# microsoft/SEAL

Measured on AMD Instinct MI355X. Metric: CKKS multiply+relinearize+rescale ciphertexts/sec @ N=2^16, L=16, higher is better.
Workload: dtype u64

## Files before the change

### seal_amd/csrc/ntt2_kernels.hip

```cpp
#include "ntt2_device.h"
#include <algorithm>
#include <atomic>
#include <mutex>
#include <cstdlib>
#include <type_traits>
#include <vector>



namespace sealhip
{
    namespace
    {

        template <bool FP, int D1, int ICLS = 0, bool PACK = false>
        __device__ __forceinline__ void fwd_p1_body(const FwdArgs &a, unsigned prime, unsigned comp, unsigned outer, uint64_t *lds, unsigned tile)
        {
            typedef Field<FP> F;
            typedef Geo<D1> G;
            const unsigned tid = threadIdx.x, cg = tile;
            const typename F::Mod m = F::make_mod(ld_uniform_mod(&a.t.mods[prime]), ld_uniform_fpd(&a.t.fpd[prime]));
            const typename F::tw_t *tab = tw_table<FP>(a.t, false, prime);
            SrcMap sm{ 0, 0, 0, 0 };
            const uint64_t *in0;
            size_t in_stride;
            if (a.src)
            {
                in0 = a.src + ((size_t)(comp % a.src_ncomp) << G::n);
                in_stride = a.src_outer_stride;
                sm.mode = a.src_mode;
                sm.half = a.src_half;
                sm.src_q = a.src_q;
                sm.fix = a.src_mode >= 2 ? a.src_fix[comp] : 0;
            }
            else
            {
                in0 = a.data + ((size_t)comp << G::n);
                in_stride = a.outer_stride;
            }
            const unsigned c = tid & (G::C - 1), rbl = tid >> G::LC;
            in0 += cg * G::C + c;
            TwRegs<FP> tw;
            p1_load_tw<FP, D1>(tw, tab, tid);
            uint64_t nxt[16];
            auto fetch = [&](unsigned z) {
                const uint64_t *in = in0 + (size_t)z * in_stride;
#pragma unroll
                for (int e = 0; e < 16; e++)
                {
                    const unsigned ra = e >> (4 - G::rA), rbh = e & ((1 << (4 - G::rA)) - 1);
                    const unsigned R = ra * 16 + (rbh << G::rA) + rbl;
#ifdef SEALHIP_P1_NOLOAD
                    nxt[e] = (uint64_t)(tid * 16 + e + z * 4099u + R) & 0xFFFFFFFFFFFFull;
#else
                    nxt[e] = a.src ? in[(size_t)R * 256] : mid_ld<16>(in + (size_t)R * 256);
#endif
                }
            };
            const unsigned ostride = gridDim.z;
            fetch(outer);
            for (; outer < a.nouter; outer += ostride)
            {
                typename F::elem x[16];
#pragma unroll
                for (int e = 0; e < 16; e++)
                    x[e] = map_src<FP>(nxt[e], sm, m);
                prio_phase<2>();
                if (outer + ostride < a.nouter)
                    fetch(outer + ostride);
                prio_phase<1>();
                uint64_t *mid_tr = a.mid + (((size_t)outer * a.ncomp + comp) << G::n);
#ifndef SEALHIP_P1_PLAIN_LEAN
#define SEALHIP_P1_PLAIN_LEAN 0
#endif
                p1_tile<FP, D1, 256, SEALHIP_P1_PLAIN_LEAN && FP && G::rA == 4, ICLS, PACK>(x, m, tab, tw, lds, mid_tr, cg, tid);
            }
        }

        template <int D1, int CLS>
#ifndef SEALHIP_PACK_WAVES_P1
#define SEALHIP_PACK_WAVES_P1 3
#endif
        __global__ void __launch_bounds__(kThreads, CLS == 5 ? SEALHIP_PACK_WAVES_P1 : CLS == 1 ? SEALHIP_FP_WAVES_P1 : 2) ntt2_fwd_p1(FwdArgs a)
        {
            HIP_DYNAMIC_SHARED(uint64_t, lds)
            const Blk blk = spread_blocks();
            const unsigned comp = blk.y + a.comp0, outer = blk.z;
            const unsigned prime = SHL_UNIFORM(a.comp_prime ? a.comp_prime[comp] : a.prime_first + comp);
            if constexpr (CLS == 5)
                fwd_p1_body<true, D1, 0, D1 == 8>(a, prime, comp, outer, lds, blk.tile);
            else if constexpr (CLS == 1)
                fwd_p1_body<true, D1>(a, prime, comp, outer, lds, blk.tile);
            else if constexpr (CLS == 0)
                with_int_class(a.t, prime, [&](auto ic) { fwd_p1_body<false, D1, decltype(ic)::value>(a, prime, comp, outer, lds, blk.tile); });
            else if (a.t.fpd[prime].qi)
                fwd_p1_body<true, D1>(a, prime, comp, outer, lds, blk.tile);
            else
                fwd_p1_body<false, D1, 2>(a, prime, comp, outer, lds, blk.tile);
        }

        template <bool FP, int D1, bool HOIST = false, bool HOIST_LDS = false, int ICLS = 0, bool PACK = false>
        __device__ __forceinline__ void fwd_p2_body(const FwdArgs &a, unsigned prime, unsigned comp, unsigned outer, uint64_t *lds, unsigned tile)
        {
            typedef Field<FP> F;
            typedef Geo<D1> G;
            const unsigned tid = threadIdx.x, hg = tile;
            const typename F::Mod m = F::make_mod(ld_uniform_mod(&a.t.mods[prime]), ld_uniform_fpd(&a.t.fpd[prime]));
            const typename F::tw_t *tab = tw_table<FP>(a.t, false, prime);
            const uint64_t *mid0 = a.mid + ((size_t)comp << G::n) + ((size_t)hg << 12) + mid_lane(tid);
            uint64_t *lds_wave = lds + (tid >> 6) * (4 * kRowWords);
            uint64_t nxt[16];
            auto fetch = [&](unsigned z) {
                const uint64_t *mp = mid0 + (((size_t)z * a.ncomp) << G::n);
#pragma unroll
                for (int e = 0; e < 16; e++)
                    nxt[e] = mid_ld<4>(mp + e * kMidRow);
            };
            constexpr bool packed = PACK;
            static_assert(!PACK || (FP && D1 == 8), "the packed intermediate is defined for the double-precision pass at N = 2^16");
            [[maybe_unused]] const uint64_t *pk0 = a.mid + ((size_t)comp << G::n) + (size_t)(hg * 16 + (tid >> 4)) * kPackBlock + (tid & 15);
            [[maybe_unused]] auto fetch_packed = [&](unsigned z) {
                const uint64_t *mp = pk0 + (((size_t)z * a.ncomp) << G::n);
#if SEALHIP_PACK_VEC16
                const uint64_t *m2 = mp + (tid & 15);
#pragma unroll
                for (int j = 0; j < 6; j++)
                    mid_ld2<4>(m2 + j * 32, nxt[2 * j], nxt[2 * j + 1]);
                nxt[12] = mid_ld<4>(mp + 192);
#else
#pragma unroll
                for (int k = 0; k < 13; k++)
                    nxt[k] = mid_ld<4>(mp + k * 16);
#endif
            };
            const unsigned ostride = gridDim.z;
            TwRegs<FP> pre_a, pre_b;
            const typename F::tw_t *twa = nullptr;
            if constexpr (HOIST_LDS)
            {
                static_assert(FP, "double-precision back end only");
                double *la = reinterpret_cast<double *>(lds + kLds2Words);
                stage_twa<D1>(la, tab, hg, tid);
                twa = la;
                const unsigned h = hg * 16 + (tid >> 4), v = tid & 15;
                load_tw<FP, 4>(pre_b, tab, [&](int t) { return (1u << (D1 + 4 + t)) + ((h * 16 + v) << t); });
                __syncthreads();
            }
            else if constexpr (HOIST)
                p2_load_tw<FP, D1>(pre_a, pre_b, tab, hg, tid);
            if constexpr (packed)
                fetch_packed(outer);
            else
                fetch(outer);
            for (; outer < a.nouter; outer += ostride)
            {
// ... 116 lines not shown
            const int mode = t2.x.halves_added ? 3 : 2;
            const SrcMap s1{ mode, a.src_half, a.src_q, a.src_fix[comp] }, s2{ mode, t2.x.src2_half, t2.x.src2_q, t2.x.src2_fix[comp] };
            const ShoupOp pm = t2.x.pmul[comp];
            const uint64_t q = a.t.mods[prime].q;
            const unsigned c = tid & (G::C - 1), rbl = tid >> G::LC;
            const size_t col = (size_t)cg * G::C + c;
            TwRegs<FP> tw;
            p1_load_tw<FP, D1>(tw, tab, tid);
            const unsigned ostride = gridDim.z;
            for (; outer < a.nouter; outer += ostride)
            {
                const uint64_t *in1 = a.src + (size_t)outer * a.src_outer_stride + col;
                const uint64_t *in2 = ((outer & 1) ? t2.x.src2_1 : t2.x.src2_0) + (size_t)(outer >> 1) * t2.x.src2_stride + col;
                uint64_t n1[16], n2[16];
#pragma unroll
                for (int e = 0; e < 16; e++)
                {
                    const unsigned ra = e >> (4 - G::rA), rbh = e & ((1 << (4 - G::rA)) - 1);
                    const unsigned R = ra * 16 + (rbh << G::rA) + rbl;
                    n1[e] = in1[(size_t)R * 256];
                    n2[e] = in2[(size_t)R * 256];
                }
                typename F::elem x[16];
                if constexpr (FP)
                {
                    const double pinv = pm.w > q / 2 ? -(double)(q - pm.w) : (double)pm.w;
                    const double f1 = fp_from_u52(s1.fix), f2 = fp_from_u52(s2.fix);
                    const bool u_small = !(s2.src_q >> 52);
#pragma unroll
                    for (int e = 0; e < 16; e++)
                    {
                        const uint64_t r1 = mode == 3 ? n1[e] : csub(n1[e] + s1.half, s1.src_q), r2 = mode == 3 ? n2[e] : csub(n2[e] + s2.half, s2.src_q);
                        const double v = F::from_any(r1, m) + f1, u = (u_small ? fp_from_u52(r2) : F::from_any(r2, m)) + f2;
                        x[e] = fp_mulmod(v, pinv, m.q, m.qinv) + u;
                        F::fix(x[e], m);
                    }
                }
                else
                {
#pragma unroll
                    for (int e = 0; e < 16; e++)
                    {
                        const typename F::elem v = map_src<FP>(n1[e], s1, m), u = map_src<FP>(n2[e], s2, m);
                        x[e] = mul_shoup(v, pm.w, pm.wq, q) + u;
                    }
                }
                uint64_t *mid_tr = a.mid + (((size_t)outer * a.ncomp + comp) << G::n);
                p1_tile<FP, D1, 256, FP && G::rA == 4, ICLS>(x, m, tab, tw, lds, mid_tr, cg, tid);
            }
        }

        template <bool FP, int D1, int ICLS>
        __device__ __forceinline__ void tail2_p2_body(const Tail2Args &t2, unsigned prime, unsigned comp, unsigned outer, uint64_t *lds, unsigned tile)
        {
            typedef Field<FP> F;
            typedef Geo<D1> G;
            const FwdArgs &a = t2.f;
            const unsigned tid = threadIdx.x, hg = tile;
            const typename F::Mod m = F::make_mod(ld_uniform_mod(&a.t.mods[prime]), ld_uniform_fpd(&a.t.fpd[prime]));
            const typename F::tw_t *tab = tw_table<FP>(a.t, false, prime);
            const uint64_t *mid0 = a.mid + ((size_t)comp << G::n) + ((size_t)hg << 12) + mid_lane(tid);
            uint64_t *lds_wave = lds + (tid >> 6) * (4 * kRowWords);
            const uint64_t q = a.t.mods[prime].q;
            const ShoupOp mul = a.epi_mul[comp], pm = t2.x.pmul[comp];
            [[maybe_unused]] const double pm_fp = pm.w > q / 2 ? -(double)(q - pm.w) : (double)pm.w;
            [[maybe_unused]] const double mul_fp = mul.w > q / 2 ? -(double)(q - mul.w) : (double)mul.w;
            const size_t row0 = ((size_t)comp << G::n) + ((size_t)(hg * 16 + (tid >> 6) * 4) << 8);
            uint64_t nxt[16];
            auto fetch = [&](unsigned z) {
                const uint64_t *mp = mid0 + (((size_t)z * a.ncomp) << G::n);
#pragma unroll
                for (int e = 0; e < 16; e++)
                    nxt[e] = mid_ld<4>(mp + e * kMidRow);
            };
            const unsigned ostride = gridDim.z;
            fetch(outer);
            for (; outer < a.nouter; outer += ostride)
            {
                typename F::elem x[16];
#pragma unroll
                for (int e = 0; e < 16; e++)
                    x[e] = F::unraw(nxt[e]);
                if (outer + ostride < a.nouter)
                    fetch(outer + ostride);
                const uint64_t *A = a.epi_a + (size_t)outer * a.epi_a_stride + row0;
                const uint64_t *C = ((outer & 1) ? t2.x.c1 : t2.x.c0) + (size_t)(outer >> 1) * t2.x.c_stride + row0;
                const bool folded = t2.x.a_has_c;
                uint64_t av[16], cv[16];
#pragma unroll
                for (int k = 0; k < 16; k++)
                {
                    const unsigned off = (k >> 2) * 256 + (k & 3) * 64 + (tid & 63);
                    av[k] = mid_ld<16>(A + off);
                    cv[k] = folded ? 0 : mid_ld<16>(C + off);
                }
                p2_tile<FP, D1, false, false, false, false, false, ICLS, kP1Out<ICLS, D1>>(x, m, tab, nullptr, nullptr, lds_wave, hg, tid);
                uint64_t val[16];
                uint64_t *O = ((outer & 1) ? a.epi_out1 : a.epi_out0) + (size_t)(outer >> 1) * a.epi_out_stride + row0;
                if constexpr (FP)
                {
#pragma unroll
                    for (int e = 0; e < 16; e++)
                        val[e] = F::raw(x[e]);
                    emit_rows_k(val, lds_wave, tid, [&](int k, unsigned off, uint64_t tv) {
                        const double s = folded ? fp_from_u52(av[k]) : fp_mulmod(fp_from_u52(av[k]), pm_fp, m.q, m.qinv) + fp_from_u52(cv[k]);
                        const double r = fp_mulmod(s - fp_from_bits(tv), mul_fp, m.q, m.qinv);
                        O[off] = fp_to_canon(fp_fix(r, m.q, m.qinv), m);
                    });
                }
                else
                {
#pragma unroll
                    for (int e = 0; e < 16; e++)
                        val[e] = fwd_out_lazy<FP, ICLS, kP2Out<ICLS, D1>>(x[e], m);
                    emit_rows_k(val, lds_wave, tid, [&](int k, unsigned off, uint64_t tv) {
                        const uint64_t s = folded ? av[k] : add_mod(mul_shoup(av[k], pm.w, pm.wq, q), cv[k], q);
                        O[off] = mul_shoup(s + 4 * q - tv, mul.w, mul.wq, q);
                    });
                }
            }
        }

        template <int D1, int CLS>
        __global__ void __launch_bounds__(kThreads, 2) ntt2_tail2_p1(Tail2Args a)
        {
            HIP_DYNAMIC_SHARED(uint64_t, lds)
            const Blk blk = spread_blocks();
            const unsigned comp = blk.y + a.f.comp0, outer = blk.z;
            const unsigned prime = SHL_UNIFORM(a.f.prime_first + comp);
            if constexpr (CLS == 1)
                tail2_p1_body<true, D1, 0>(a, prime, comp, outer, lds, blk.tile);
            else if constexpr (CLS == 0)
                with_int_class(a.f.t, prime, [&](auto ic) { tail2_p1_body<false, D1, decltype(ic)::value>(a, prime, comp, outer, lds, blk.tile); });
            else if (a.f.t.fpd[prime].qi)
                tail2_p1_body<true, D1, 0>(a, prime, comp, outer, lds, blk.tile);
            else
                tail2_p1_body<false, D1, 2>(a, prime, comp, outer, lds, blk.tile);
        }
        template <int D1, int CLS>
        __global__ void __launch_bounds__(kThreads, 2) ntt2_tail2_p2(Tail2Args a)
        {
            HIP_DYNAMIC_SHARED(uint64_t, lds)
            const Blk blk = spread_blocks();
            const unsigned comp = blk.y + a.f.comp0, outer = blk.z;
            const unsigned prime = SHL_UNIFORM(a.f.prime_first + comp);
            if constexpr (CLS == 1)
                tail2_p2_body<true, D1, 0>(a, prime, comp, outer, lds, blk.tile);
            else if constexpr (CLS == 0)
                with_int_class(a.f.t, prime, [&](auto ic) { tail2_p2_body<false, D1, decltype(ic)::value>(a, prime, comp, outer, lds, blk.tile); });
            else if (a.f.t.fpd[prime].qi)
                tail2_p2_body<true, D1, 0>(a, prime, comp, outer, lds, blk.tile);
            else
                tail2_p2_body<false, D1, 2>(a, prime, comp, outer, lds, blk.tile);
        }

        struct InvArgs
        {
            uint64_t *data;
            size_t outer_stride;
            const uint64_t *src;
            size_t src_outer_stride;
            uint64_t *mid;
            const uint32_t *comp_prime;
            int cls_hint;
            unsigned prime_first;
            unsigned ncomp;
            unsigned comp0;
            unsigned nouter;
            int lazy;
            uint64_t out_add;
            const uint64_t *prod_x, *prod_y;
            unsigned prod_batch, prod_outer0;
            uint64_t *prod_out;
            size_t prod_out_stride;
            uint32_t src_gal;
            NttTables t;
        };

        template <int ICLS>
        constexpr int kInvE1 = inv_phase_exp<ICLS>(0, 4, 0);
        template <int ICLS>
        constexpr int kInvE2 = inv_phase_exp<ICLS>(kInvE1<ICLS>, 4, 0);
        template <int ICLS>
        constexpr int kInvE3 = inv_phase_exp<ICLS>(kInvE2<ICLS>, 4, 0);

        template <bool FP, int D1, int ICLS = 2>
        __device__ __forceinline__ void inv_pa_body(const InvArgs &a, unsigned prime, unsigned comp, unsigned outer, uint64_t *lds, unsigned tile)
        {
            typedef Field<FP> F;
            typedef Geo<D1> G;
            const unsigned tid = threadIdx.x, hg = tile;
            const unsigned v = tid & 15, u = tid >> 4, ul = u & 3;
            const unsigned h = hg * 16 + u;
            const typename F::Mod m = F::make_mod(ld_uniform_mod(&a.t.mods[prime]), ld_uniform_fpd(&a.t.fpd[prime]));
            const typename F::tw_t *tab = tw_table<FP>(a.t, true, prime);
            uint64_t *lds_wave = lds + (tid >> 6) * (4 * kRowWords);
            uint64_t raw[16];
            typename F::elem x[16];
            bool have_x = false;
            const size_t rows = ((size_t)comp << G::n) + ((size_t)(hg * 16 + (tid >> 6) * 4) << 8);
            if (a.prod_x)
            {
                const unsigned go = outer + a.prod_outer0, pp = go / a.prod_batch, b = go - pp * a.prod_batch;
                const size_t plane = (size_t)a.prod_batch * a.src_outer_stride, off = (size_t)b * a.src_outer_stride + rows;
                [[maybe_unused]] const ModDesc md = ld_uniform_mod(&a.t.mods[prime]);
                uint64_t rb[16];
                load_rows(raw, lds_wave, a.prod_x + (pp == 2 ? plane : 0) + off, tid);
                load_rows(rb, lds_wave, a.prod_y + (pp == 0 ? 0 : plane) + off, tid);
                if constexpr (FP)
                {
#pragma unroll
                    for (int e = 0; e < 16; e++)
                        x[e] = fp_mulmod(fp_from_u52(raw[e]), fp_from_u52(rb[e]), m.q, m.qinv);
                    if (pp == 1)
                    {
                        uint64_t rc[16];
                        load_rows(rc, lds_wave, a.prod_x + plane + off, tid);
                        load_rows(rb, lds_wave, a.prod_y + off, tid);
#pragma unroll
                        for (int e = 0; e < 16; e++)
                            x[e] += fp_mulmod(fp_from_u52(rc[e]), fp_from_u52(rb[e]), m.q, m.qinv);
                    }
#pragma unroll
                    for (int e = 0; e < 16; e++)
                        F::fix(x[e], m);
                    if (a.prod_out)
                    {
#pragma unroll
                        for (int e = 0; e < 16; e++)
                            raw[e] = fp_to_canon(x[e], m);
                        store_rows(raw, lds_wave, a.prod_out + (size_t)outer * a.prod_out_stride + rows, tid);
                    }
                    have_x = true;
                }
                else
                {
#pragma unroll
                    for (int e = 0; e < 16; e++)
                        raw[e] = mul_mod(raw[e], rb[e], md);
                    if (pp == 1)
                    {
                        uint64_t rc[16];
                        load_rows(rc, lds_wave, a.prod_x + plane + off, tid);
                        load_rows(rb, lds_wave, a.prod_y + off, tid);
#pragma unroll
                        for (int e = 0; e < 16; e++)
                            raw[e] = add_mod(raw[e], mul_mod(rc[e], rb[e], md), md.q);
                    }
                    if (a.prod_out)
                        store_rows(raw, lds_wave, a.prod_out + (size_t)outer * a.prod_out_stride + rows, tid);
                }
            }
            else if (a.src_gal)
                load_rows_galois(raw, lds_wave, a.src + (size_t)outer * a.src_outer_stride + ((size_t)comp << G::n), (hg * 16 + (tid >> 6) * 4) << 8, a.src_gal, G::n, tid);
            else
                load_rows(raw, lds_wave, a.src + (size_t)outer * a.src_outer_stride + rows, tid);
            if (!have_x)
            {
#pragma unroll
                for (int e = 0; e < 16; e++)
                {
                    x[e] = F::from_canon(raw[e], m);
                    F::fix(x[e], m);
                }
            }
            {
                TwRegs<FP> tw;
                load_tw<FP, 4>(tw, tab, [&](int t) { return (1u << (D1 + 4 + t)) + ((h * 16 + v) << t); });
                phase_inv<FP, 4, 0, ICLS, 0>(x, m, [&](int t, int g) { return tw.get((1 << t) + g); });
            }
#pragma unroll
            for (int e = 0; e < 16; e++)
                F::fix(x[e], m);
#pragma unroll
            for (int e = 0; e < 16; e++)
                lds_wave[ul * kRowWords + v * 18 + e] = F::raw(x[e]);
            __builtin_amdgcn_wave_barrier();
#pragma unroll
            for (int e = 0; e < 16; e++)
                x[e] = F::unraw(lds_wave[ul * kRowWords + e * 18 + v]);
            {
                TwRegs<FP> tw;
                load_tw<FP, 4>(tw, tab, [&](int t) { return (1u << (D1 + t)) + (h << t); });
                phase_inv<FP, 4, 0, ICLS, kInvE1<ICLS>>(x, m, [&](int t, int g) { return tw.get((1 << t) + g); });
            }
#pragma unroll
            for (int e = 0; e < 16; e++)
                F::fix(x[e], m);
            uint64_t *mid_tr = a.mid + (((size_t)outer * a.ncomp + comp) << G::n) + ((size_t)hg << 12);
#pragma unroll
            for (int e = 0; e < 16; e++)
                mid_st<8>(mid_tr + e * 256 + tid, F::raw(x[e]));
        }

        template <int D1, int CLS>
        __global__ void __launch_bounds__(kThreads) ntt2_inv_pa(InvArgs a)
        {
            HIP_DYNAMIC_SHARED(uint64_t, lds)
            const Blk blk = spread_blocks();
            const unsigned comp = blk.y + a.comp0, outer = blk.z;
            const unsigned prime = SHL_UNIFORM(a.comp_prime ? a.comp_prime[comp] : a.prime_first + comp);
            if constexpr (CLS == 1)
                inv_pa_body<true, D1>(a, prime, comp, outer, lds, blk.tile);
            else if constexpr (CLS == 0)
                with_int_class(a.t, prime, [&](auto ic) { inv_pa_body<false, D1, decltype(ic)::value>(a, prime, comp, outer, lds, blk.tile); });
            else if (a.t.fpd[prime].qi)
// ... 1087 lines not shown
            {
                const size_t p = i & (N - 1), slab = i >> n_log;
                const unsigned comp = (unsigned)(slab % L);
                const size_t poly = slab / L, digit = poly >> 1;
                const unsigned k = (unsigned)(poly & 1);
                const size_t hg = p >> 12;
                const unsigned e = (unsigned)(p >> 8) & 15, tid = (unsigned)p & 255;
                size_t nat = (hg << 12) + ((size_t)(tid >> 4) << 8) + ((tid & 15) << 4) + e;
                const uint64_t v = in[(slab << n_log) + nat];
                uint64_t *o = out + ((digit * off[L] + off[comp]) << n_log);
                if (fpd[comp].qi)
                {
                    double d = fp_from_u52(v);
                    if (v > fpd[comp].qi / 2)
                        d -= fpd[comp].q;
                    o[2 * p + k] = fp_to_bits(d);
                }
                else
                {
                    typedef unsigned __int128 u128;
                    const ModDesc md = mods[comp];
                    const u128 vr = (u128)v * md.ratio_hi + (((u128)v * md.ratio_lo) >> 64);
                    uint64_t est = vr > (u128)~(uint64_t)0 ? ~(uint64_t)0 : (uint64_t)vr;
                    u128 rem = ((u128)v << 64) - (u128)est * md.q;
                    while (rem >= md.q)
                    {
                        rem -= md.q;
                        est++;
                    }
                    o += (size_t)k << (n_log + 1);
                    o[2 * p] = v;
                    o[2 * p + 1] = est;
                }
            }
        }

        __global__ void __launch_bounds__(kThreads) key_unlayout_kernel(
            const uint64_t *in, uint64_t *out, const FpDesc *fpd, unsigned L, unsigned n_log, size_t polys)
        {
            __shared__ unsigned off[kMaxKeyComps + 1];
            key_offsets(off, fpd, L);
            const size_t N = (size_t)1 << n_log;
            const size_t total = polys * L * N;
            for (size_t i = blockIdx.x * (size_t)kThreads + threadIdx.x; i < total; i += (size_t)gridDim.x * kThreads)
            {
                const size_t p = i & (N - 1), slab = i >> n_log;
                const unsigned comp = (unsigned)(slab % L);
                const size_t poly = slab / L, digit = poly >> 1;
                const unsigned k = (unsigned)(poly & 1);
                const size_t hg = p >> 12;
                const unsigned e = (unsigned)(p >> 8) & 15, tid = (unsigned)p & 255;
                const size_t nat = (hg << 12) + ((size_t)(tid >> 4) << 8) + ((tid & 15) << 4) + e;
                const uint64_t *o = in + ((digit * off[L] + off[comp]) << n_log);
                uint64_t v;
                if (fpd[comp].qi)
                {
                    double d = fp_from_bits(o[2 * p + k]);
                    if (d < 0)
                        d += fpd[comp].q;
                    v = (uint64_t)d;
                }
                else
                    v = o[((size_t)k << (n_log + 1)) + 2 * p];
                out[(slab << n_log) + nat] = v;
            }
        }

        struct CompRun
        {
            unsigned c0, nc;
            int cls;
        };
        std::vector<CompRun> comp_runs(const NttTables &t, const uint32_t *comp_prime, unsigned prime_first, unsigned ncomp, int cls_hint = -1)
        {
            std::vector<CompRun> runs;
            if (comp_prime && (cls_hint == 0 || cls_hint == 1))
            {
                runs.push_back(CompRun{ 0, ncomp, cls_hint });
                return runs;
            }
            static const bool split = !shl_ab_getenv("SEALHIP_NTT_NOSPLIT");
            unsigned c = 0;
            while (c < ncomp)
            {
                int cls = 2;
                unsigned e = ncomp;
                if (split && !comp_prime && t.fp_host)
                {
                    cls = t.fp_host[prime_first + c] ? 1 : 0;
                    e = c + 1;
                    while (e < ncomp && (t.fp_host[prime_first + e] ? 1 : 0) == cls)
                        e++;
                }
                runs.push_back(CompRun{ c, e - c, cls });
                c = e;
            }
            return runs;
        }

        struct SideStream
        {
            hipStream_t stream = nullptr;
            hipEvent_t fork = nullptr, join = nullptr;
            bool ok = false;
            SideStream()
            {
                ok = !shl_ab_getenv("SEALHIP_NTT_NOFORK") && hipStreamCreateWithFlags(&stream, hipStreamNonBlocking) == hipSuccess &&
                     hipEventCreateWithFlags(&fork, hipEventDisableTiming) == hipSuccess &&
                     hipEventCreateWithFlags(&join, hipEventDisableTiming) == hipSuccess;
            }
        };
        SideStream &side_stream()
        {
            static thread_local SideStream s;
            return s;
        }
        template <class RunFn>
        hipError_t launch_runs(const std::vector<CompRun> &runs, hipStream_t s, RunFn run, bool may_fork = true)
        {
            size_t longest = 0;
            for (size_t i = 1; i < runs.size(); i++)
                if (runs[i].nc > runs[longest].nc)
                    longest = i;
            SideStream &ss = side_stream();
            const bool fork = may_fork && runs.size() > 1 && ss.ok;
            hipError_t e;
            if (fork)
            {
                if ((e = hipEventRecord(ss.fork, s)) != hipSuccess || (e = hipStreamWaitEvent(ss.stream, ss.fork, 0)) != hipSuccess)
                    return e;
                for (size_t i = 0; i < runs.size(); i++)
                    if (i != longest && (e = run(runs[i], ss.stream)) != hipSuccess)
                        return e;
                if ((e = hipEventRecord(ss.join, ss.stream)) != hipSuccess)
                    return e;
            }
            for (size_t i = 0; i < runs.size(); i++)
                if ((!fork || i == longest) && (e = run(runs[i], s)) != hipSuccess)
                    return e;
            if (fork && (e = hipStreamWaitEvent(s, ss.join, 0)) != hipSuccess)
                return e;
            return hipSuccess;
        }

#ifndef SEALHIP_FUSED_FORK14
#define SEALHIP_FUSED_FORK14 1
#endif
        inline bool fused_int()
        {
            static const bool on = !shl_ab_getenv("SEALHIP_NTT_NOFUSED_INT");
            return on;
        }

        template <int D1>
        hipError_t launch_fwd(const FwdArgs &a, unsigned nouter, hipStream_t s)
        {
            typedef Geo<D1> G;
            unsigned per = G::TILES * a.ncomp;
#ifndef SEALHIP_NTT_WG_TARGET
#define SEALHIP_NTT_WG_TARGET 8192
#endif
            unsigned chunks = (SEALHIP_NTT_WG_TARGET + per - 1) / per;
            if (const char *f = shl_ab_getenv("SEALHIP_NTT_CHUNKS"))
                chunks = (unsigned)std::atoi(f) ? (unsigned)std::atoi(f) : 1;
            if (chunks > nouter)
                chunks = nouter;
            if (chunks > 65535)
                chunks = 65535;
            size_t l1 = G::rA > 0 ? G::lds1_words * 8 : 8;
            bool fused = false;
            unsigned fchunks = 1;
            if constexpr (D1 == 5 || D1 == 6)
            {
                static const bool fused_ok = !shl_ab_getenv("SEALHIP_NTT_NOFUSED");
                if (fused_ok && (!a.src || a.src_mode == 0) && a.epi == 0)
                {
                    static bool raised = false;
                    if (!raised)
                    {
                        if (hipFuncSetAttribute(reinterpret_cast<const void *>(&ntt2_fwd_fused2<D1, 1>), hipFuncAttributeMaxDynamicSharedMemorySize, (int)FusedGeo<D1>::lds_bytes) != hipSuccess ||
                            hipFuncSetAttribute(reinterpret_cast<const void *>(&ntt2_fwd_fused2<D1, 0>), hipFuncAttributeMaxDynamicSharedMemorySize, (int)(FusedGeo<D1, 2>::lds_bytes)) != hipSuccess)
                            return hipErrorInvalidValue;
                        raised = true;
                    }
                    fused = true;
                    const unsigned want = D1 == 5 ? 2048 : 1024;
                    fchunks = (want + a.ncomp - 1) / a.ncomp;
                    if (const char *f = std::getenv("SEALHIP_NTT_FCHUNKS"))
                        fchunks = (unsigned)std::atoi(f) ? (unsigned)std::atoi(f) : 1;
                    if (fchunks > nouter)
                        fchunks = nouter;
                    if (fchunks > 65535)
                        fchunks = 65535;
                }
            }
            return launch_runs(comp_runs(a.t, a.comp_prime, a.prime_first, a.ncomp, a.cls_hint), s, [&](const CompRun &r, hipStream_t st) {
                FwdArgs g = a;
                g.comp0 = r.c0;
#ifndef SEALHIP_MID_PACK
#define SEALHIP_MID_PACK 1
#endif
                g.mid_pack = SEALHIP_MID_PACK && D1 == 8 && r.cls == 1 && a.epi == 0 && chunks < nouter ? 1 : 0;
                if constexpr (D1 == 5 || D1 == 6)
                {
                    if (fused && r.cls == 1)
                    {
                        hipLaunchKernelGGL((ntt2_fwd_fused2<D1, 1>), dim3(1, r.nc, fchunks), dim3(FusedGeo<D1>::TEAMS * kThreads), FusedGeo<D1>::lds_bytes, st, g);
                        return hipGetLastError();
                    }
                    if (fused && r.cls == 0 && fused_int())
                    {
                        constexpr size_t lds_int = FusedGeo<D1, 2>::lds_bytes;
                        hipLaunchKernelGGL((ntt2_fwd_fused2<D1, 0>), dim3(1, r.nc, fchunks), dim3(FusedGeo<D1>::TEAMS * kThreads), lds_int, st, g);
                        return hipGetLastError();
                    }
                }
                dim3 grid(G::TILES, r.nc, chunks);
                if constexpr (D1 == 8)
                {
                    if (r.cls == 1 && !a.src && a.epi == 0 && a.ring)
                    {
                        const unsigned z = ntt2_ring_teams(r.nc, nouter);
                        if (z && ntt2_ring_run_words(r.nc, z) <= a.ring_words && ntt2_ring_stream_ok(st))
                        {
                            const NttRingRun run{ a.data, a.outer_stride, a.comp_prime, a.prime_first, a.ncomp, r.c0, r.nc, nouter, a.lazy, z, a.ring, a.ring_words };
                            return ntt2_ring_launch(a.t, run, st);
                        }
                    }
                }
                if constexpr (D1 == 8)
                {
                    if (g.mid_pack)
                    {
                        hipLaunchKernelGGL((ntt2_fwd_p1<D1, 5>), grid, dim3(kThreads), l1, st, g);
                        hipError_t ep = hipGetLastError();
                        if (ep != hipSuccess)
                            return ep;
                        hipLaunchKernelGGL((ntt2_fwd_p2<D1, 5>), grid, dim3(kThreads), (kLds2Words + 240) * 8, st, g);
                        return hipGetLastError();
                    }
                }
                if (r.cls == 1)
                    hipLaunchKernelGGL((ntt2_fwd_p1<D1, 1>), grid, dim3(kThreads), l1, st, g);
                else if (r.cls == 0)
                    hipLaunchKernelGGL((ntt2_fwd_p1<D1, 0>), grid, dim3(kThreads), l1, st, g);
                else
                    hipLaunchKernelGGL((ntt2_fwd_p1<D1, 2>), grid, dim3(kThreads), l1, st, g);
                hipError_t e = hipGetLastError();
                if (e != hipSuccess)
                    return e;
                static const int p2_hoist = shl_ab_getenv("SEALHIP_P2_HOIST") ? std::atoi(shl_ab_getenv("SEALHIP_P2_HOIST")) : 4;
                if (r.cls == 1 && a.epi == 0 && chunks < nouter && p2_hoist == 4)
                    hipLaunchKernelGGL((ntt2_fwd_p2<D1, 4>), grid, dim3(kThreads), (kLds2Words + 240) * 8, st, g);
                else if (r.cls == 1 && a.epi == 0 && chunks < nouter && p2_hoist == 3)
                    hipLaunchKernelGGL((ntt2_fwd_p2<D1, 3>), grid, dim3(kThreads), kLds2Words * 8, st, g);
                else if (r.cls == 1)
                    hipLaunchKernelGGL((ntt2_fwd_p2<D1, 1>), grid, dim3(kThreads), kLds2Words * 8, st, g);
                else if (r.cls == 0)
                    hipLaunchKernelGGL((ntt2_fwd_p2<D1, 0>), grid, dim3(kThreads), kLds2Words * 8, st, g);
                else
                    hipLaunchKernelGGL((ntt2_fwd_p2<D1, 2>), grid, dim3(kThreads), kLds2Words * 8, st, g);
                return hipGetLastError();
            }, !(fused && fused_int()) || (D1 == 6 && SEALHIP_FUSED_FORK14));
        }

        template <int D1>
        hipError_t launch_tail2(const Tail2Args &a, unsigned nouter, hipStream_t s)
        {
            typedef Geo<D1> G;
            unsigned per = G::TILES * a.f.ncomp;
#ifndef SEALHIP_TAIL2_WG_TARGET
#define SEALHIP_TAIL2_WG_TARGET 4096
#endif
            unsigned chunks = (SEALHIP_TAIL2_WG_TARGET + per - 1) / per;
            if (chunks > nouter)
                chunks = nouter;
            if (chunks > 65535)
                chunks = 65535;
            const size_t l1 = G::rA > 0 ? G::lds1_words * 8 : 8;
            return launch_runs(comp_runs(a.f.t, nullptr, a.f.prime_first, a.f.ncomp), s, [&](const CompRun &r, hipStream_t st) {
                Tail2Args g = a;
                g.f.comp0 = r.c0;
                dim3 grid(G::TILES, r.nc, chunks);
                if (r.cls == 1)
                    hipLaunchKernelGGL((ntt2_tail2_p1<D1, 1>), grid, dim3(kThreads), l1, st, g);
                else if (r.cls == 0)
                    hipLaunchKernelGGL((ntt2_tail2_p1<D1, 0>), grid, dim3(kThreads), l1, st, g);
                else
                    hipLaunchKernelGGL((ntt2_tail2_p1<D1, 2>), grid, dim3(kThreads), l1, st, g);
                hipError_t e = hipGetLastError();
                if (e != hipSuccess)
                    return e;
                if (r.cls == 1)
                    hipLaunchKernelGGL((ntt2_tail2_p2<D1, 1>), grid, dim3(kThreads), kLds2Words * 8, st, g);
                else if (r.cls == 0)
                    hipLaunchKernelGGL((ntt2_tail2_p2<D1, 0>), grid, dim3(kThreads), kLds2Words * 8, st, g);
                else
                    hipLaunchKernelGGL((ntt2_tail2_p2<D1, 2>), grid, dim3(kThreads), kLds2Words * 8, st, g);
                return hipGetLastError();
            });
        }

        template <int D1>
        hipError_t launch_inv(const InvArgs &a, unsigned nouter, hipStream_t s)
        {
            typedef Geo<D1> G;
            bool fused = false;
            unsigned fchunks = 1;
            if constexpr (D1 == 5 || D1 == 6)
            {
                static const bool fused_ok = !shl_ab_getenv("SEALHIP_NTT_NOFUSED");
                if (fused_ok && !a.prod_x && !a.src_gal)
                {
                    static bool raised = false;
                    if (!raised)
                    {
                        if (hipFuncSetAttribute(reinterpret_cast<const void *>(&ntt2_inv_fused2<D1, 1>), hipFuncAttributeMaxDynamicSharedMemorySize, (int)FusedGeo<D1>::lds_bytes) != hipSuccess ||
                            hipFuncSetAttribute(reinterpret_cast<const void *>(&ntt2_inv_fused2<D1, 0>), hipFuncAttributeMaxDynamicSharedMemorySize, (int)(FusedGeo<D1, 2>::lds_bytes)) != hipSuccess)
                            return hipErrorInvalidValue;
                        raised = true;
                    }
                    fused = true;
                    const unsigned want = D1 == 5 ? 2048 : 1024;
                    fchunks = (want + a.ncomp - 1) / a.ncomp;
                    if (D1 == 5 && nouter / 4 > fchunks)
                        fchunks = nouter / 4;
                    if (const char *f = std::getenv("SEALHIP_NTT_FCHUNKS"))
                        fchunks = (unsigned)std::atoi(f) ? (unsigned)std::atoi(f) : 1;
                    if (fchunks > nouter)
                        fchunks = nouter;
                    if (fchunks > 65535)
                        fchunks = 65535;
                }
            }
            return launch_runs(comp_runs(a.t, a.comp_prime, a.prime_first, a.ncomp, a.cls_hint), s, [&](const CompRun &r, hipStream_t st) {
                InvArgs g = a;
                g.comp0 = r.c0;
                g.nouter = nouter;
                if constexpr (D1 == 5 || D1 == 6)
                {
                    if (fused && r.cls == 1)
                    {
                        hipLaunchKernelGGL((ntt2_inv_fused2<D1, 1>), dim3(1, r.nc, fchunks), dim3(FusedGeo<D1>::TEAMS * kThreads), FusedGeo<D1>::lds_bytes, st, g);
                        return hipGetLastError();
                    }
                    if (fused && r.cls == 0 && fused_int())
                    {
                        constexpr size_t lds_int = FusedGeo<D1, 2>::lds_bytes;
                        hipLaunchKernelGGL((ntt2_inv_fused2<D1, 0>), dim3(1, r.nc, fchunks), dim3(FusedGeo<D1>::TEAMS * kThreads), lds_int, st, g);
                        return hipGetLastError();
                    }
                }
                dim3 grid(G::TILES, r.nc, nouter);
                if (r.cls == 1)
                    hipLaunchKernelGGL((ntt2_inv_pa<D1, 1>), grid, dim3(kThreads), kLds2Words * 8, st, g);
                else if (r.cls == 0)
                    hipLaunchKernelGGL((ntt2_inv_pa<D1, 0>), grid, dim3(kThreads), kLds2Words * 8, st, g);
                else
                    hipLaunchKernelGGL((ntt2_inv_pa<D1, 2>), grid, dim3(kThreads), kLds2Words * 8, st, g);
                hipError_t e = hipGetLastError();
                if (e != hipSuccess)
                    return e;
                static const char *skip_env = shl_ab_getenv("SEALHIP_AB_SKIP_INV_PB");
                static long skip_after = skip_env ? std::atol(skip_env) : -1;
                static std::atomic<long> inv_launches{ 0 };
                if (skip_after >= 0 && inv_launches.fetch_add(1) >= skip_after)
                    return (hipError_t)hipSuccess;
                if (r.cls == 1)
                    hipLaunchKernelGGL((ntt2_inv_pb<D1, 1>), grid, dim3(kThreads), G::lds1_words * 8, st, g);
                else if (r.cls == 0)
                    hipLaunchKernelGGL((ntt2_inv_pb<D1, 0>), grid, dim3(kThreads), G::lds1_words * 8, st, g);
                else
                    hipLaunchKernelGGL((ntt2_inv_pb<D1, 2>), grid, dim3(kThreads), G::lds1_words * 8, st, g);
                return hipGetLastError();
            }, !(fused && fused_int()) || (D1 == 6 && SEALHIP_FUSED_FORK14));
        }

        template <int D1>
        hipError_t launch_ks(const Ks1Args &a1, const Ks2Args &a2, unsigned batch, unsigned n_int, hipStream_t s, int order1, bool no_class_fork)
        {
            typedef Geo<D1> G;
            if (a1.ntargets == 0)
                return hipSuccess;
            const size_t l1 = G::rA > 0 ? G::lds1_words * 8 : 8;
            const unsigned vbatch = batch * a1.parts;
            const unsigned groups = vbatch * G::TILES;
            const unsigned n_fp = a1.ntargets - n_int;
            const size_t l2_fp = kLds2Words * 8 + (240 + 3840) * sizeof(double);
            const size_t l2_int = kLds2Words * 8 + (240 + (SEALHIP_KS2_INT_TWB3 ? 2048 : 0)) * sizeof(ShoupOp);
            if (n_int && l2_int > 65536)
            {
                static bool raised_int = false;
                if (!raised_int)
                {
                    if (hipFuncSetAttribute(reinterpret_cast<const void *>(&ks2_kernel<D1, 0>), hipFuncAttributeMaxDynamicSharedMemorySize, (int)l2_int) != hipSuccess)
                        return hipErrorInvalidValue;
                    raised_int = true;
                }
            }
            if (n_fp && l2_fp > 65536)
            {
                static bool raised = false;
                if (!raised)
                {
                    if (hipFuncSetAttribute(reinterpret_cast<const void *>(&ks2_kernel<D1, 1>), hipFuncAttributeMaxDynamicSharedMemorySize, (int)l2_fp) != hipSuccess)
                        return hipErrorInvalidValue;
                    raised = true;
                }
            }
            auto run_class = [&](bool fp, hipStream_t st) -> hipError_t {
                const unsigned t0 = fp ? n_int : 0, nt = fp ? n_fp : n_int;
                if (!nt)
                    return hipSuccess;
                Ks1Args c1 = a1;
                c1.targets = a1.targets + 2 * t0;
                c1.ntargets = nt;
                const dim3 g1(((groups + 7) / 8) * nt * 8);
                static const char *order_env = shl_ab_getenv("SEALHIP_KS1_ORDER");
                const unsigned g1t = batch * (a1.j1 - a1.j0) * G::TILES;
                const bool digit_resident = order_env ? order_env[0] == '1' : order1 >= 0 ? (order1 == 1 && a1.parts == 1) : (a1.parts == 1 && g1t >= 4096);
                if (digit_resident && fp)
                {
                    const unsigned char *small = a1.tb.fp_host;
                    for (unsigned ja = a1.j0; ja < a1.j1;)
                    {
                        const bool sm = small && small[ja];
                        unsigned jb = ja + 1;
                        while (jb < a1.j1 && (small && small[jb]) == sm)
                            jb++;
                        Ks1Args cr = c1;
                        cr.j0 = ja;
                        cr.j1 = jb;
                        const dim3 gr(batch * (jb - ja) * G::TILES);
                        if (sm)
                            hipLaunchKernelGGL((ks1t_kernel<true, D1, true>), gr, dim3(kThreads), l1, st, cr);
                        else
                            hipLaunchKernelGGL((ks1t_kernel<true, D1, false>), gr, dim3(kThreads), l1, st, cr);
// ... 287 lines not shown
```

Measured before the change: 10150.

## Add source-resident NTT pass-1 kernel that reuses loaded source across target primes

Adds a pass-1 kernel for the forward NTT and the folded tail that loads a source tile into registers once, then loops over all target primes (components) in a single workgroup. Each prime gets its own mapping, multiply and first-pass butterflies. Before, each component's workgroup reloaded the same source coefficients from global memory. It is used when the run has more than one target of a single class and enough workgroups. The cost is a serialized per-workgroup loop over components, less parallelism per launch, and more register pressure.

```diff
diff --git a/seal_amd/csrc/ntt2_kernels.hip b/seal_amd/csrc/ntt2_kernels.hip
--- a/seal_amd/csrc/ntt2_kernels.hip
+++ b/seal_amd/csrc/ntt2_kernels.hip
@@ -1,6 +1,7 @@
 #include "ntt2_device.h"
 #include <algorithm>
 #include <atomic>
+#include <cstdio>
 #include <mutex>
 #include <cstdlib>
 #include <type_traits>
@@ -423,6 +424,129 @@
                 tail2_p2_body<true, D1, 0>(a, prime, comp, outer, lds, blk.tile);
             else
                 tail2_p2_body<false, D1, 2>(a, prime, comp, outer, lds, blk.tile);
+        }
+
+        __device__ __forceinline__ uint64_t resident_word(uint64_t v)
+        {
+#if defined(__HIP_DEVICE_COMPILE__)
+            asm volatile("" : "+v"(v));
+#endif
+            return v;
+        }
+
+        template <bool FP, int D1, bool TWO, bool SMALL2>
+        __device__ __forceinline__ void src_p1t_body(const Tail2Args &t2, unsigned nc, uint64_t *lds)
+        {
+            static_assert(!SMALL2 || (FP && TWO), "SMALL2 is a property of the double-precision launch of the folded tail");
+            typedef Field<FP> F;
+            typedef Geo<D1> G;
+            const FwdArgs &a = t2.f;
+            const unsigned tid = threadIdx.x;
+            const unsigned grp = blockIdx.x;
+            if (grp >= a.nouter * G::TILES)
+                return;
+            const unsigned cg = grp % G::TILES, outer = grp / G::TILES;
+            const unsigned c = tid & (G::C - 1), rbl = tid >> G::LC;
+            const size_t col = (size_t)cg * G::C + c;
+            const uint64_t *in1 = a.src + (size_t)outer * a.src_outer_stride + col;
+            [[maybe_unused]] const uint64_t *in2 = nullptr;
+            if constexpr (TWO)
+                in2 = ((outer & 1) ? t2.x.src2_1 : t2.x.src2_0) + (size_t)(outer >> 1) * t2.x.src2_stride + col;
+            uint64_t r1[16];
+            [[maybe_unused]] uint64_t r2[16];
+#pragma unroll
+            for (int e = 0; e < 16; e++)
+            {
+                const unsigned ra = e >> (4 - G::rA), rbh = e & ((1 << (4 - G::rA)) - 1);
+                const unsigned R = ra * 16 + (rbh << G::rA) + rbl;
+                r1[e] = in1[(size_t)R * 256];
+                if constexpr (TWO)
+                    r2[e] = in2[(size_t)R * 256];
+            }
+            const bool add_half = TWO ? !t2.x.halves_added : a.src_mode == 2;
+            if (add_half)
+            {
+#pragma unroll
+                for (int e = 0; e < 16; e++)
+                {
+                    r1[e] = csub(r1[e] + a.src_half, a.src_q);
+                    if constexpr (TWO)
+                        r2[e] = csub(r2[e] + t2.x.src2_half, t2.x.src2_q);
+                }
+            }
+            if constexpr (SMALL2)
+            {
+#pragma unroll
+                for (int e = 0; e < 16; e++)
+                    r2[e] = fp_to_bits(fp_from_u52(r2[e]));
+            }
+#pragma nounroll
+            for (unsigned it = 0; it < nc; it++)
+            {
+                const unsigned comp = a.comp0 + it;
+                const unsigned prime = SHL_UNIFORM(a.comp_prime ? a.comp_prime[comp] : a.prime_first + comp);
+                uint64_t *mid_tr = a.mid + (((size_t)outer * a.ncomp + comp) << G::n);
+                auto one = [&](auto ic) {
+                    constexpr int ICLS = decltype(ic)::value;
+                    const typename F::Mod m = F::make_mod(ld_uniform_mod(&a.t.mods[prime]), ld_uniform_fpd(&a.t.fpd[prime]));
+                    const typename F::tw_t *tab = tw_table<FP>(a.t, false, prime);
+                    TwRegs<FP> tw;
+                    p1_load_tw<FP, D1>(tw, tab, tid);
+                    const SrcMap s1{ 3, 0, 0, a.src_fix[comp] };
+                    typename F::elem x[16];
+                    if constexpr (!TWO)
+                    {
+#pragma unroll
+                        for (int e = 0; e < 16; e++)
+                            x[e] = map_src<FP>(resident_word(r1[e]), s1, m);
+                        p1_tile<FP, D1, 256, SEALHIP_P1_PLAIN_LEAN && FP && G::rA == 4, ICLS>(x, m, tab, tw, lds, mid_tr, cg, tid);
+                    }
+                    else
+                    {
+                        const ShoupOp pm = t2.x.pmul[comp];
+                        const uint64_t q = a.t.mods[prime].q;
+                        if constexpr (FP)
+                        {
+                            const double pinv = pm.w > q / 2 ? -(double)(q - pm.w) : (double)pm.w;
+                            const double f1 = fp_from_u52(s1.fix), f2 = fp_from_u52(t2.x.src2_fix[comp]);
+#pragma unroll
+                            for (int e = 0; e < 16; e++)
+                            {
+                                const double v = F::from_any(resident_word(r1[e]), m) + f1;
+                                const double u = (SMALL2 ? fp_from_bits(r2[e]) : F::from_any(resident_word(r2[e]), m)) + f2;
+                                x[e] = fp_mulmod(v, pinv, m.q, m.qinv) + u;
+                                F::fix(x[e], m);
+                            }
+                        }
+                        else
+                        {
+                            const SrcMap s2{ 3, 0, 0, t2.x.src2_fix[comp] };
+#pragma unroll
+                            for (int e = 0; e < 16; e++)
+                            {
+                                const typename F::elem v = map_src<FP>(resident_word(r1[e]), s1, m), u = map_src<FP>(resident_word(r2[e]), s2, m);
+                                x[e] = mul_shoup(v, pm.w, pm.wq, q) + u;
+                            }
+                        }
+                        p1_tile<FP, D1, 256, FP && G::rA == 4, ICLS>(x, m, tab, tw, lds, mid_tr, cg, tid);
+                    }
+                };
+                if constexpr (FP)
+                    one(std::integral_constant<int, 0>());
+                else
+                    with_int_class(a.t, prime, one);
+            }
+        }
+
+#ifndef SEALHIP_SRC_P1T_FP2_WGS
+#define SEALHIP_SRC_P1T_FP2_WGS 2
+#endif
+        template <int D1, int CLS, bool TWO, bool SMALL2 = false>
+        __global__ void __launch_bounds__(kThreads, SMALL2 ? SEALHIP_SRC_P1T_FP2_WGS : 2) ntt2_src_p1t(Tail2Args a, unsigned nc)
+        {
+            static_assert(CLS == 0 || CLS == 1, "single-class runs only");
+            HIP_DYNAMIC_SHARED(uint64_t, lds)
+            src_p1t_body<CLS == 1, D1, TWO, SMALL2>(a, nc, lds);
         }
 
         struct InvArgs
@@ -1816,6 +1940,42 @@
             return on;
         }
 
+#ifndef SEALHIP_SRC_P1T_MIN_WGS
+#define SEALHIP_SRC_P1T_MIN_WGS 512
+#endif
+        inline bool src_resident(unsigned tiles, unsigned nouter, const CompRun &r)
+        {
+            static const char *order_env = std::getenv("SEALHIP_TAIL_P1_ORDER");
+            static const char *min_env = shl_ab_getenv("SEALHIP_TAIL_P1_MIN_WGS");
+            static const bool trace = shl_ab_getenv("SEALHIP_TAIL_P1_TRACE") != nullptr;
+            static const size_t min_wgs = min_env ? (size_t)std::atol(min_env) : (size_t)SEALHIP_SRC_P1T_MIN_WGS;
+            bool yes = false;
+            if (r.cls != 0 && r.cls != 1)
+                yes = false;
+            else if (order_env && (order_env[0] == '0' || order_env[0] == '1'))
+                yes = order_env[0] == '1';
+            else
+                yes = r.nc > 1 && (size_t)tiles * nouter >= min_wgs;
+            if (trace)
+                std::fprintf(stderr, "[tail] pass 1 %s (%u tiles x %u items, %u targets of class %d)\n", yes ? "source-resident" : "target-resident",
+                             tiles, nouter, r.nc, r.cls);
+            return yes;
+        }
+        template <int D1, bool TWO>
+        hipError_t launch_src_p1t(const Tail2Args &g, const CompRun &r, unsigned nouter, hipStream_t st)
+        {
+            typedef Geo<D1> G;
+            const size_t l1 = G::rA > 0 ? G::lds1_words * 8 : 8;
+            const dim3 grid(G::TILES * nouter);
+            if (r.cls == 1 && TWO && !(g.x.src2_q >> 52))
+                hipLaunchKernelGGL((ntt2_src_p1t<D1, 1, TWO, TWO>), grid, dim3(kThreads), l1, st, g, r.nc);
+            else if (r.cls == 1)
+                hipLaunchKernelGGL((ntt2_src_p1t<D1, 1, TWO>), grid, dim3(kThreads), l1, st, g, r.nc);
+            else
+                hipLaunchKernelGGL((ntt2_src_p1t<D1, 0, TWO>), grid, dim3(kThreads), l1, st, g, r.nc);
+            return hipGetLastError();
+        }
+
         template <int D1>
         hipError_t launch_fwd(const FwdArgs &a, unsigned nouter, hipStream_t s)
         {
@@ -1904,7 +2064,13 @@
                         return hipGetLastError();
                     }
                 }
-                if (r.cls == 1)
+                if (a.src && (a.src_mode == 2 || a.src_mode == 3) && a.src_ncomp == 1 && src_resident(G::TILES, nouter, r))
+                {
+                    hipError_t e1 = launch_src_p1t<D1, false>(Tail2Args{ g, NttTail2{} }, r, nouter, st);
+                    if (e1 != hipSuccess)
+                        return e1;
+                }
+                else if (r.cls == 1)
                     hipLaunchKernelGGL((ntt2_fwd_p1<D1, 1>), grid, dim3(kThreads), l1, st, g);
                 else if (r.cls == 0)
                     hipLaunchKernelGGL((ntt2_fwd_p1<D1, 0>), grid, dim3(kThreads), l1, st, g);
@@ -1946,7 +2112,13 @@
                 Tail2Args g = a;
                 g.f.comp0 = r.c0;
                 dim3 grid(G::TILES, r.nc, chunks);
-                if (r.cls == 1)
+                if (src_resident(G::TILES, nouter, r))
+                {
+                    hipError_t e1 = launch_src_p1t<D1, true>(g, r, nouter, st);
+                    if (e1 != hipSuccess)
+                        return e1;
+                }
+                else if (r.cls == 1)
                     hipLaunchKernelGGL((ntt2_tail2_p1<D1, 1>), grid, dim3(kThreads), l1, st, g);
                 else if (r.cls == 0)
                     hipLaunchKernelGGL((ntt2_tail2_p1<D1, 0>), grid, dim3(kThreads), l1, st, g);
```

Result: faster. 10320, median of 6 (+1.6%).
